# unknownue/puflow

Measured on AMD Instinct MI355X. Metric: patches/sec x4 2048->8192 (PU1K discrete, eval), higher is better.
Workload: dtype f32 (split-fp16 MFMA products, fp32 accumulate); 1 GPU; BASELINE configs[1]: PU1K discrete x4 inference, 32 x 2048-pt patches per GPU (fp32-parity mode); patches_per_gpu=32, total_batch=32, npoint=2048

## Files before the change

puflow_amd/csrc/edgeconv.hip:

```cpp
#include <hip/hip_runtime.h>
#include "pf_api_internal.h"
#include "pf_mfma.h"

namespace {

struct EcArgs {
    const float* pq;
    const float* xyz;
    const float* tab;
    const int* idx;
    const f4* wg;
    float* out;
    int T;
    int N;
    int chunk;
    int ntiles;
    const u4* pqf_w;
    const float* pqf_bias;
    const float* pqf_scales;
    float* pqf_out;
};

template <int ODIM>
__device__ __forceinline__ void pqf_stage(u4* hb, int ch, int pt, float v) {
// ... 328 lines not shown
            for (int o = 0; o < OCH; ++o)
#pragma unroll
                for (int p = 0; p < P; ++p)
                    m[p][ob0 + o] = fmaxf(fmaxf(acc[p][o].x, acc[p][o].y), fmaxf(acc[p][o].z, acc[p][o].w));
        });
#pragma unroll
        for (int p = 0; p < P; ++p) {
            const float o0 = pf_rsmax16(pf_rsmax32(m[p][0], m[p][1]), pf_rsmax32(m[p][2], m[p][3]));
            const float o1 = pf_rsmax16(pf_rsmax32(m[p][4], m[p][5]), pf_rsmax32(m[p][6], m[p][7]));
            const int ch = 16 * blkq + col;
            const float* pr = reinterpret_cast<const float*>(plds[wave * P + p]);
            const float p0 = pr[G * NCONV + ch], p1 = pr[G * NCONV + 64 + ch];
            const float h0 = fmaf(o0, EC4_OUT_INV, p0), h1 = fmaf(o1, EC4_OUT_INV, p1);
            if (pt0 + p < a.T) {
                float* o = a.out + (size_t)gout[p] * ODIM + ch;
                o[0] = h0;
                o[64] = h1;
            }
            if constexpr (PQF) {
                u4* hbt = hb + pqf.nst * ((ODIM / 32) * 2 * 64);
                pqf_stage<ODIM>(hbt, ch, wave * P + p, h0);
                pqf_stage<ODIM>(hbt, ch + 64, wave * P + p, h1);
            }
        }
        if constexpr (PQF) {
            pqf.push(pf_xcd_tile(v, a.chunk) * NW * P);
            if (pqf.nst == PQF_NT || vn >= vend) {
                __syncthreads();
                pqf_gemm<ODIM, 2 * S, NW>(a, hb, pqf.nst, pqf.tpt, __builtin_amdgcn_readfirstlane(wave), lane);
                __syncthreads();
                pqf.nst = 0;
            }
        }
        v = vn;
    }
}

template <int P, int NW, int DBG = 0, bool PQF = false>
int launch4(const EcArgs& a0, hipStream_t s) {
    EcArgs a = a0;
    a.ntiles = (a.T + NW * P - 1) / (NW * P);
    a.chunk = (a.ntiles + 7) / 8;
    int grid = 8 * a.chunk;
    if (grid > 256) grid = 256;
    hipLaunchKernelGGL((edgeconv4_kernel<P, NW, DBG, PQF>), dim3(grid), dim3(NW * 64), 0, s, a);
    return pf_last_launch_status();
}

template <int ODIM, bool C3, int P, int NW, bool PQF = false>
__global__ __launch_bounds__(NW * 64) void edgeconv1n_kernel(EcArgs a) {
    static_assert(!PQF || NW * P == 16, "the fused P|Q GEMM takes a workgroup tile of 16 points as one MFMA column tile");
    constexpr int NCONV = 4, S = 16 * NCONV + ODIM, SB = S / 16, OBO = ODIM / 16;
    constexpr int PQ_ROWS = ODIM == 32 ? 256 : 512;
    constexpr int FO = 4, FT = FO + OBO * 2, NWF = FT + (C3 ? SB : 0);
    constexpr int ROWB = 2 * S * 4;
    static_assert(OBO == 2 || OBO == 4, "reduce-scatter below is written for 2 or 4 output blocks");
    const int lane = threadIdx.x & 63, wave = threadIdx.x >> 6;
    const int col = lane & 15, q = lane >> 4;
    __shared__ u4 wlds[NWF * 128];
    __shared__ float plds[C3 ? 1 : NW * P][C3 ? 1 : S];
    __shared__ u4 hb[PQF ? PQF_NT * (ODIM / 32) * 2 * 64 : 1];
    PqfState pqf;
    pf_stage_lds(wlds, reinterpret_cast<const u4*>(a.wg), NWF * 128);
    __syncthreads();
    const PfW2Lds ws{wlds, lane};
    const __amdgpu_buffer_rsrc_t rs = __builtin_amdgcn_make_buffer_rsrc(const_cast<float*>(C3 ? a.xyz : a.pq), 0, 0x7fffffff, 0x00020000);

    for (int v = blockIdx.x; v < 8 * a.chunk; v += gridDim.x) {
        const int tile = pf_xcd_tile(v, a.chunk);
        if (tile >= a.ntiles) continue;
        const int pt0 = (tile * NW + wave) * P;
        int gi[P], vQ[P], vO[P][4];
        PfPairN e[P][1];
#pragma unroll
        for (int p = 0; p < P; ++p) {
            int g = pt0 + p;
            g = g < a.T ? g : a.T - 1;
            g = __builtin_amdgcn_readfirstlane(g);
            gi[p] = g;
            const int bN = (g / a.N) * a.N;
            const int jc = bN + a.idx[(size_t)g * 16 + col];
            if constexpr (C3) {
                float xi[3], xj[3];
#pragma unroll
                for (int c = 0; c < 3; ++c) {
                    xi[c] = a.xyz[(size_t)g * 3 + c];
                    xj[c] = a.xyz[(size_t)jc * 3 + c];
                }
                const f4 z4 = pf_splat(0.f);
                const f4 e0 = {xi[0], xi[1], xi[2], xj[0]}, e1 = {xj[1], xj[2], 0.f, 1.f};
                e[p][0] = pf_pairn(q == 0 ? e0 : z4, q == 0 ? e1 : z4);
            } else {
                const int4 j4 = *reinterpret_cast<const int4*>(a.idx + (size_t)g * 16 + 4 * q);
                vQ[p] = jc * ROWB + (S + 4 * q) * 4;
                vO[p][0] = (bN + j4.x) * ROWB + (S + 16 * NCONV + col) * 4;
                vO[p][1] = (bN + j4.y) * ROWB + (S + 16 * NCONV + col) * 4;
                vO[p][2] = (bN + j4.z) * ROWB + (S + 16 * NCONV + col) * 4;
                vO[p][3] = (bN + j4.w) * ROWB + (S + 16 * NCONV + col) * 4;
                if (lane * 2 < S) {
                    typedef float f2 __attribute__((ext_vector_type(2)));
                    const f2 pv = *reinterpret_cast<const f2*>(a.pq + (size_t)g * (2 * S) + lane * 2);
                    *reinterpret_cast<f2*>(&plds[wave * P + p][lane * 2]) = pv;
                }
            }
        }
        f4 pre[P][NCONV];
        f4 outi[P][OBO];
        if constexpr (C3) {
#pragma unroll
            for (int p = 0; p < P; ++p) {
#pragma unroll
                for (int b = 0; b < NCONV; ++b) pre[p][b] = pf_splat(0.f);
#pragma unroll
                for (int b = 0; b < OBO; ++b) outi[p][b] = pf_splat(0.f);
            }
            pf_mmn<false, NCONV, 1, 1>(ws, FT, e, pre);
            pf_mmn<true, OBO, 1, 1>(ws, FT + NCONV, e, outi);
        } else {
#pragma unroll
            for (int b = 0; b < NCONV; ++b)
#pragma unroll
                for (int p = 0; p < P; ++p)
                    pre[p][b] = __builtin_bit_cast(f4, __builtin_amdgcn_raw_buffer_load_b128(rs, vQ[p], b * 64, 0));
#pragma unroll
            for (int b = 0; b < OBO; ++b)
#pragma unroll
                for (int p = 0; p < P; ++p)
#pragma unroll
                    for (int r = 0; r < 4; ++r)
                        outi[p][b][r] = __builtin_bit_cast(float, __builtin_amdgcn_raw_buffer_load_b32(rs, vO[p][r], b * 64, 0));
#pragma unroll
            for (int b = 0; b < NCONV; ++b)
#pragma unroll
                for (int p = 0; p < P; ++p) pre[p][b] += *reinterpret_cast<const f4*>(&plds[wave * P + p][16 * b + 4 * q]);
        }

        PfPairN fp[P][2];
        f4 last[P];
#pragma unroll
        for (int p = 0; p < P; ++p) {
            last[p] = pf_lrelu(pre[p][0], 0.05f);
            fp[p][0] = pf_pairn(last[p], pf_splat(0.f));
        }
        pf_static_for<1, NCONV>([&](auto tc) {
            constexpr int t = decltype(tc)::value;
            constexpr int CPT = (t + 1) / 2, F0 = (t / 2) * ((t + 1) / 2);
            f4 acc[P][1];
#pragma unroll
            for (int p = 0; p < P; ++p) acc[p][0] = pre[p][t];
            pf_mmn<false, 1, CPT, CPT>(ws, F0, fp, acc);
#pragma unroll
            for (int p = 0; p < P; ++p) {
                const f4 f = pf_lrelu(acc[p][0], 0.05f);
                if constexpr (t % 2 == 1) fp[p][t / 2] = pf_pairn(last[p], f);
                else fp[p][t / 2] = pf_pairn(f, pf_splat(0.f));
                last[p] = f;
            }
        });
        pf_mmn<true, OBO, 2, 2>(ws, FO, fp, outi);
#pragma unroll
        for (int p = 0; p < P; ++p) {
            float m[OBO];
#pragma unroll
            for (int b = 0; b < OBO; ++b) m[b] = fmaxf(fmaxf(outi[p][b].x, outi[p][b].y), fmaxf(outi[p][b].z, outi[p][b].w));
            float o;
            int ch;
            if constexpr (OBO == 4) {
                o = pf_rsmax16(pf_rsmax32(m[0], m[1]), pf_rsmax32(m[2], m[3]));
                ch = 16 * (((q & 1) << 1) | (q >> 1)) + col;
            } else {
                const float n = pf_rsmax32(m[0], m[1]);
                o = pf_rsmax16(n, n);
                ch = 16 * (q >> 1) + col;
            }
            float pv = 0.f;
            if constexpr (!C3) pv = plds[wave * P + p][16 * NCONV + ch];
            const float hv = fmaf(o, EC4_OUT_INV, pv);
            if (pt0 + p < a.T && (OBO == 4 || (q & 1) == 0))
                a.out[(size_t)gi[p] * ODIM + ch] = hv;
            if constexpr (PQF) {
                if (OBO == 4 || (q & 1) == 0) pqf_stage<ODIM>(hb + pqf.nst * ((ODIM / 32) * 2 * 64), ch, wave * P + p, hv);
            }
        }
        if constexpr (PQF) {
            pqf.push(tile * NW * P);
            if (pqf.nst == PQF_NT) {
                __syncthreads();
                pqf_gemm<ODIM, PQ_ROWS, NW>(a, hb, pqf.nst, pqf.tpt, __builtin_amdgcn_readfirstlane(wave), lane);
                __syncthreads();
                pqf.nst = 0;
            }
        }
    }
    if constexpr (PQF) {
        if (pqf.nst > 0) {
            __syncthreads();
            pqf_gemm<ODIM, PQ_ROWS, NW>(a, hb, pqf.nst, pqf.tpt, __builtin_amdgcn_readfirstlane(wave), lane);
        }
    }
}

template <int ODIM, bool C3, int P, int NW, bool PQF = false>
int launch1n(const EcArgs& a0, hipStream_t s) {
// ... 152 lines not shown
```

puflow_amd/csrc/interp.hip:

```cpp
#include <hip/hip_runtime.h>
#include "pf_api_internal.h"
#include "pf_mfma.h"

#ifndef PF_INTERP_P
#define PF_INTERP_P 1
#endif
#ifndef PF_INTERP_NW
#define PF_INTERP_NW 12
#endif

namespace {

struct InterpArgs {
    const float* xyz;
    const float* z;
    const int* idx;
    const float* w;
    long long off[15];
    float* u;
    float* aw;
    int T, N, ntiles, R;
    int per;
    int contiguous;
};

template <int P, int NW, bool BIG = false>
__global__ __launch_bounds__(NW * 64) void interp_kernel(InterpArgs a) {
    constexpr int R = 4;
    const int lane = threadIdx.x & 63, wave = threadIdx.x >> 6;
    const int col = lane & 15, q = lane >> 4;
    const int ps = col >> 3, k = col & 7;
    constexpr int L_DT = 0, L_ET = 4, L_WT = 12, L_D3 = 20, L_EC = 28, L_D6 = 44, L_W3 = 60, L_END = 76;
    __shared__ u4 wl[L_END * 128];
    {
        auto stage = [&](int f0, int nf, long long off) {
            const u4* src = reinterpret_cast<const u4*>(a.w + off);
            pf_stage_lds(wl + f0 * 128, src, nf * 128);
        };
        if (a.contiguous) stage(L_DT, L_END, a.off[0]);
        else {
            stage(L_DT, 4, a.off[0]); stage(L_ET, 8, a.off[5]); stage(L_WT, 8, a.off[8]); stage(L_D3, 8, a.off[1]);
            stage(L_EC, 16, a.off[6]); stage(L_D6, 16, a.off[3]); stage(L_W3, 16, a.off[9]);
        }
        __syncthreads();
    }
    const PfW2Lds wsDT{wl + L_DT * 128, lane}, wsET{wl + L_ET * 128, lane}, wsWT{wl + L_WT * 128, lane},
        wsD3{wl + L_D3 * 128, lane}, wsEC{wl + L_EC * 128, lane}, wsD6{wl + L_D6 * 128, lane}, wsW3{wl + L_W3 * 128, lane};
    const PfW2BufD<4> wsW0(a.w + a.off[7], lane);
    const PfW2BufD<2> wsW6(a.w + a.off[BIG ? 13 : 11], lane);

    const float* sc = a.w + a.off[4];
    const float iDT = sc[0], iD3 = sc[1], iW1 = sc[2], iEC = sc[3], iW3 = sc[4], iW6 = sc[5];

    const int wt_end = min((int)(blockIdx.x + 1) * a.per, a.ntiles);
    for (int wt = blockIdx.x * a.per + wave; wt < wt_end; wt += NW) {
        const int pt0 = wt * P * 2;
        int gi[P], gj[P];
        bool ok[P];
        PfPairN e[P][1];
#pragma unroll
        for (int p = 0; p < P; ++p) {
            const int g = pt0 + p * 2 + ps;
            ok[p] = g < a.T;
            gi[p] = ok[p] ? g : a.T - 1;
            gj[p] = (gi[p] / a.N) * a.N + a.idx[(size_t)gi[p] * 16 + k];
            float xi[3], xj[3];
#pragma unroll
            for (int c = 0; c < 3; ++c) {
                xi[c] = a.xyz[(size_t)gi[p] * 3 + c];
                xj[c] = a.xyz[(size_t)gj[p] * 3 + c];
            }
            const float v0 = xi[0] - xj[0], v1 = xi[1] - xj[1], v2 = xi[2] - xj[2];
            const float nrm = sqrtf(__fadd_rn(__fadd_rn(__fmul_rn(v0, v0), __fmul_rn(v1, v1)), __fmul_rn(v2, v2)));
            const f4 z4 = pf_splat(0.f);
            const f4 e0 = {xi[0], xi[1], xi[2], xj[0]}, e1 = {xj[1], xj[2], nrm, 1.f};
            e[p][0] = pf_pairn(q == 0 ? e0 : z4, q == 0 ? e1 : z4);
        }

        f4 w1[P][8];
        {
            PfPairN fp[P][4];
            f4 last[P];
            {
                f4 acc[P][1];
#pragma unroll
                for (int p = 0; p < P; ++p) acc[p][0] = pf_splat(0.f);
                pf_mmn<false, 1, 1, 1>(wsET, 0, e, acc);
#pragma unroll
                for (int p = 0; p < P; ++p) {
                    last[p] = pf_lrelu(acc[p][0] * iEC, 0.05f);
                    fp[p][0] = pf_pairn(last[p], pf_splat(0.f));
                }
            }
            pf_static_for<1, 8>([&](auto tc) {
                constexpr int t = decltype(tc)::value;
                constexpr int CPT = (t + 1) / 2;
                constexpr int F0 = (t / 2) * ((t + 1) / 2);
                f4 acc[P][1];
#pragma unroll
                for (int p = 0; p < P; ++p) acc[p][0] = pf_splat(0.f);
                pf_mmn<false, 1, 1, 1>(wsET, t, e, acc);
                pf_mmn<false, 1, CPT, CPT>(wsEC, F0, fp, acc);
#pragma unroll
                for (int p = 0; p < P; ++p) {
                    const f4 f = pf_lrelu(acc[p][0] * iEC, 0.05f);
                    if constexpr (t % 2 == 1) fp[p][t / 2] = pf_pairn(last[p], f);
                    else fp[p][t / 2] = pf_pairn(f, pf_splat(0.f));
                    last[p] = f;
                }
            });
#pragma unroll
            for (int ob = 0; ob < 8; ++ob)
#pragma unroll
                for (int p = 0; p < P; ++p) w1[p][ob] = pf_splat(0.f);
            pf_mmn<false, 4, 1, 1>(wsWT, 0, e, w1, 0, 0);
            pf_mmn<false, 4, 1, 1>(wsWT, 4, e, w1, 0, 4);
            pf_mmn<false, 4, 4, 4>(wsW0, 0, fp, w1, 0, 0);
            pf_mmn<false, 4, 4, 4>(wsW0, 16, fp, w1, 0, 4);
        }

        {
            f4 d[P][4];
#pragma unroll
            for (int cb = 0; cb < 4; ++cb)
#pragma unroll
                for (int p = 0; p < P; ++p) d[p][cb] = pf_splat(0.f);
            pf_mmn<false, 4, 1, 1>(wsDT, 0, e, d);
            PfPairN dp[P][2];
#pragma unroll
            for (int p = 0; p < P; ++p) {
                dp[p][0] = pf_pairn(pf_lrelu(d[p][0] * iDT, 0.01f), pf_lrelu(d[p][1] * iDT, 0.01f));
                dp[p][1] = pf_pairn(pf_lrelu(d[p][2] * iDT, 0.01f), pf_lrelu(d[p][3] * iDT, 0.01f));
            }
#pragma unroll
            for (int cb = 0; cb < 4; ++cb)
#pragma unroll
                for (int p = 0; p < P; ++p) d[p][cb] = pf_bias(a.w + a.off[2], cb, q);
            pf_mmn<false, 4, 2, 2>(wsD3, 0, dp, d);
#pragma unroll
            for (int p = 0; p < P; ++p) {
                dp[p][0] = pf_pairn(pf_lrelu(d[p][0] * iD3, 0.01f), pf_lrelu(d[p][1] * iD3, 0.01f));
                dp[p][1] = pf_pairn(pf_lrelu(d[p][2] * iD3, 0.01f), pf_lrelu(d[p][3] * iD3, 0.01f));
            }
            pf_mmn<false, 4, 2, 2>(wsD6, 0, dp, w1, 0, 0);
            pf_mmn<false, 4, 2, 2>(wsD6, 8, dp, w1, 0, 4);
        }

        f4 w3[P][BIG ? 2 : 1];
        {
            PfPairN w1p[P][4];
#pragma unroll
            for (int c = 0; c < 4; ++c)
#pragma unroll
                for (int p = 0; p < P; ++p)
                    w1p[p][c] = pf_pairn(pf_lrelu(w1[p][2 * c] * iW1, 0.01f), pf_lrelu(w1[p][2 * c + 1] * iW1, 0.01f));
            f4 w2[P][4];
#pragma unroll
            for (int ob = 0; ob < 4; ++ob)
#pragma unroll
                for (int p = 0; p < P; ++p) w2[p][ob] = pf_bias(a.w + a.off[10], ob, q);
            pf_mmn<false, 4, 4, 4>(wsW3, 0, w1p, w2);
            PfPairN w2p[P][2];
#pragma unroll
            for (int p = 0; p < P; ++p) {
                w2p[p][0] = pf_pairn(pf_lrelu(w2[p][0] * iW3, 0.01f), pf_lrelu(w2[p][1] * iW3, 0.01f));
                w2p[p][1] = pf_pairn(pf_lrelu(w2[p][2] * iW3, 0.01f), pf_lrelu(w2[p][3] * iW3, 0.01f));
            }
#pragma unroll
            for (int p = 0; p < P; ++p)
#pragma unroll
                for (int ob = 0; ob < (BIG ? 2 : 1); ++ob) w3[p][ob] = pf_bias(a.w + a.off[BIG ? 14 : 12], ob, q);
            pf_mmn<false, (BIG ? 2 : 1), 2, 2>(wsW6, 0, w2p, w3);
#pragma unroll
            for (int p = 0; p < P; ++p)
#pragma unroll
                for (int ob = 0; ob < (BIG ? 2 : 1); ++ob) w3[p][ob] = w3[p][ob] * iW6;
        }

#pragma unroll
        for (int p = 0; p < P; ++p) {
// ... 11 lines not shown
                        m = fmaxf(m, __shfl_xor(m, 1)); m = fmaxf(m, __shfl_xor(m, 2)); m = fmaxf(m, __shfl_xor(m, 4));
                        const float ex = expf(x - m);
                        float sm = ex;
                        sm += __shfl_xor(sm, 1); sm += __shfl_xor(sm, 2); sm += __shfl_xor(sm, 4);
                        const float av = ex / sm;
#pragma unroll
                        for (int c = 0; c < 3; ++c) {
                            float s = av * zj[c];
                            s += __shfl_xor(s, 1); s += __shfl_xor(s, 2); s += __shfl_xor(s, 4);
                            if (ok[p] && k == 0 && row < a.R) a.u[((size_t)gi[p] * a.R + row) * 3 + c] = s;
                        }
                    }
            } else {
                float av[R];
#pragma unroll
                for (int r = 0; r < R; ++r) {
                    const float x = w3[p][0][r];
                    float m = x;
                    m = fmaxf(m, __shfl_xor(m, 1)); m = fmaxf(m, __shfl_xor(m, 2)); m = fmaxf(m, __shfl_xor(m, 4));
                    const float ex = expf(x - m);
                    float s = ex;
                    s += __shfl_xor(s, 1); s += __shfl_xor(s, 2); s += __shfl_xor(s, 4);
                    av[r] = ex / s;
                }
                if (a.aw) {
                    if (ok[p] && q == 0) {
                        f4 o = {av[0], av[1], av[2], av[3]};
                        *reinterpret_cast<f4*>(a.aw + ((size_t)gi[p] * 8 + k) * 4) = o;
                    }
                    continue;
                }
                const float zj = a.z[(size_t)gj[p] * 3 + (q < 3 ? q : 0)];
#pragma unroll
                for (int r = 0; r < R; ++r) {
                    float s = av[r] * zj;
                    s += __shfl_xor(s, 1); s += __shfl_xor(s, 2); s += __shfl_xor(s, 4);
                    if (ok[p] && k == 0 && q < 3 && r < a.R) a.u[((size_t)gi[p] * a.R + r) * 3 + q] = s;
                }
            }
        }
    }
}

}

static int interp_launch(const float* xyz, const float* z, const int* idx16, const float* w, const long long* off,
                         float* u_out, float* aw_out, int B, int N, int R, void* stream) {
    if (B <= 0 || N < 8 || (long long)B * N > (1ll << 28)) return PF_ERR_SHAPE;
    if (R < 1 || R > 32) return PF_ERR_UNSUPPORTED;
    constexpr int NWB = 8;
    InterpArgs a{};
    a.xyz = xyz; a.z = z; a.idx = idx16; a.w = w; a.u = u_out; a.aw = aw_out; a.T = B * N; a.N = N; a.R = R;
    for (int i = 0; i < 15; ++i) a.off[i] = off[i];
    a.contiguous = off[5] == off[0] + 4 * 512 && off[8] == off[5] + 8 * 512 && off[1] == off[8] + 8 * 512 &&
                   off[6] == off[1] + 8 * 512 && off[3] == off[6] + 16 * 512 && off[9] == off[3] + 16 * 512;
    auto go = [&](auto pc, auto nwc, auto bigc) {
        constexpr int P = decltype(pc)::value, NW = decltype(nwc)::value;
        constexpr bool BIG = decltype(bigc)::value;
        a.ntiles = (a.T + P * 2 - 1) / (P * 2);
        const int wgt = (a.ntiles + NW - 1) / NW;
        const int grid = wgt < 256 ? wgt : 256;
        a.per = (a.ntiles + grid - 1) / grid;
        hipLaunchKernelGGL((interp_kernel<P, NW, BIG>), dim3(grid), dim3(NW * 64), 0, (hipStream_t)stream, a);
    };
    if (R > 4) go(std::integral_constant<int, 1>{}, std::integral_constant<int, NWB>{}, std::true_type{});
    else go(std::integral_constant<int, PF_INTERP_P>{}, std::integral_constant<int, PF_INTERP_NW>{}, std::false_type{});
    return pf_last_launch_status();
}

extern "C" int pf_interp(const float* xyz, const float* z, const int* idx16, const float* w, const long long* off,
                         float* u_out, int B, int N, int R, void* stream) {
    if (!xyz || !z || !idx16 || !w || !off || !u_out) return PF_ERR_NULL;
    return interp_launch(xyz, z, idx16, w, off, u_out, nullptr, B, N, R, stream);
}

extern "C" int pf_interp_weights(const float* xyz, const int* idx16, const float* w, const long long* off, float* aw_out,
                                 int B, int N, void* stream) {
    if (!xyz || !idx16 || !w || !off || !aw_out) return PF_ERR_NULL;
    return interp_launch(xyz, nullptr, idx16, w, off, nullptr, aw_out, B, N, 4, stream);
}
```

puflow_amd/csrc/pf_mfma.h:

```cpp
#pragma once
#include <hip/hip_runtime.h>
#include <type_traits>

typedef float f4 __attribute__((ext_vector_type(4)));

#define PF_WAVE 64

__device__ __forceinline__ f4 pf_mfma(float a, float b, f4 c) {
    return __builtin_amdgcn_mfma_f32_16x16x4f32(a, b, c, 0, 0, 0);
}

__device__ __forceinline__ f4 pf_splat(float v) { f4 r = {v, v, v, v}; return r; }

__device__ __forceinline__ f4 pf_lrelu(f4 v, float slope) {
    const f4 s = v * slope;
    f4 r;
    r.x = fmaxf(v.x, s.x); r.y = fmaxf(v.y, s.y); r.z = fmaxf(v.z, s.z); r.w = fmaxf(v.w, s.w);
    return r;
}

__device__ __forceinline__ f4 pf_relu(f4 v) {
    f4 r;
    r.x = fmaxf(v.x, 0.f); r.y = fmaxf(v.y, 0.f); r.z = fmaxf(v.z, 0.f); r.w = fmaxf(v.w, 0.f);
    return r;
// ... 34 lines not shown
        if (i + DD < NFRAG) wb[i % DD] = ws.load(frag0 + ((i + DD) / CB) * WCB + ((i + DD) % CB));
#pragma unroll
        for (int r = 0; r < 4; ++r) {
#pragma unroll
            for (int p = 0; p < P; ++p)
                acc[p][acc0 + ob] = pf_mfma(wv[r], in[p][in0 + cb][r], acc[p][acc0 + ob]);
        }
        __builtin_amdgcn_sched_barrier(0);
    }
}

typedef unsigned int u4 __attribute__((ext_vector_type(4)));

typedef _Float16 h8 __attribute__((ext_vector_type(8)));
typedef _Float16 h2 __attribute__((ext_vector_type(2)));
typedef unsigned int u2 __attribute__((ext_vector_type(2)));
constexpr float PF_LO_SCALE = 2048.f, PF_LO_INV = 1.f / 2048.f;

__device__ __forceinline__ u2 pf_split2_pair(float a, float b) {
    unsigned hb = __builtin_bit_cast(unsigned, (h2){(_Float16)a, (_Float16)b});
    asm("" : "+v"(hb));
    const h2 h = __builtin_bit_cast(h2, hb);
    const h2 l = {(_Float16)((a - (float)h.x) * PF_LO_SCALE), (_Float16)((b - (float)h.y) * PF_LO_SCALE)};
    return (u2){hb, __builtin_bit_cast(unsigned, l)};
}

struct PfPair2 { h8 h, l; };
__device__ __forceinline__ PfPair2 pf_pair2(f4 b0, f4 b1) {
    const u2 s0 = pf_split2_pair(b0.x, b0.y), s1 = pf_split2_pair(b0.z, b0.w);
    const u2 s2 = pf_split2_pair(b1.x, b1.y), s3 = pf_split2_pair(b1.z, b1.w);
    PfPair2 p;
    p.h = __builtin_bit_cast(h8, (u4){s0.x, s1.x, s2.x, s3.x});
    p.l = __builtin_bit_cast(h8, (u4){s0.y, s1.y, s2.y, s3.y});
    return p;
}

__device__ __forceinline__ f4 pf_mfma_f16(h8 a, h8 b, f4 c) {
    return __builtin_amdgcn_mfma_f32_16x16x32_f16(a, b, c, 0, 0, 0);
}

#ifndef PF_MM2_DEPTH
#define PF_MM2_DEPTH 8
#endif
#ifndef PF_W2LDS_DEPTH
#define PF_W2LDS_DEPTH 2
#endif
struct PfW2Lds {
    static constexpr int DEPTH = PF_W2LDS_DEPTH;
    const u4* base;
    int lane;
    __device__ __forceinline__ h8 load(int frag, int split) const {
        return __builtin_bit_cast(h8, base[(frag * 2 + split) * PF_WAVE + lane]);
    }
};

template <int DEPTH_>
struct PfW2BufD {
    static constexpr int DEPTH = DEPTH_;
    __amdgpu_buffer_rsrc_t rsrc;
    int voff;
    __device__ __forceinline__ PfW2BufD(const void* p, int lane)
        : rsrc(__builtin_amdgcn_make_buffer_rsrc(const_cast<void*>(p), 0, 0x7fffffff, 0x00020000)), voff(lane * 16) {}
    __device__ __forceinline__ h8 load(int frag, int split) const {
        return __builtin_bit_cast(h8, __builtin_amdgcn_raw_buffer_load_b128(rsrc, voff, (frag * 2 + split) * (PF_WAVE * 16), 0));
    }
};

struct PfW2Buf {
    static constexpr int DEPTH = PF_MM2_DEPTH;
    __amdgpu_buffer_rsrc_t rsrc;
    int voff;
    __device__ __forceinline__ PfW2Buf(const void* p, int lane)
        : rsrc(__builtin_amdgcn_make_buffer_rsrc(const_cast<void*>(p), 0, 0x7fffffff, 0x00020000)), voff(lane * 16) {}
    __device__ __forceinline__ h8 load(int frag, int split) const {
        return __builtin_bit_cast(h8, __builtin_amdgcn_raw_buffer_load_b128(rsrc, voff, (frag * 2 + split) * (PF_WAVE * 16), 0));
    }
};

template <int OB, int CP, int WCP, int D = 2, class WS2, int P, int NIN, int NACC>
__device__ __forceinline__ void pf_mm2(const WS2& ws, int frag0, const PfPair2 (&in)[P][NIN], int in0,
                                       f4 (&acc)[P][NACC], f4 (&accx)[P][NACC], int acc0) {
    constexpr int NFRAG = OB * CP;
    constexpr int DD = D < NFRAG ? D : NFRAG;
    h8 wb[DD][2];
#pragma unroll
    for (int i = 0; i < DD; ++i)
#pragma unroll
        for (int s = 0; s < 2; ++s) wb[i][s] = ws.load(frag0 + (i / CP) * WCP + (i % CP), s);
#pragma unroll
    for (int i = 0; i < NFRAG; ++i) {
        const int ob = i / CP, cp = i % CP;
        const h8 wh = wb[i % DD][0], wl = wb[i % DD][1];
        if (i + DD < NFRAG) {
            const int f = frag0 + ((i + DD) / CP) * WCP + ((i + DD) % CP);
#pragma unroll
            for (int s = 0; s < 2; ++s) wb[i % DD][s] = ws.load(f, s);
        }
#pragma unroll
        for (int p = 0; p < P; ++p) {
            f4 x = accx[p][acc0 + ob];
            x = pf_mfma_f16(wh, in[p][in0 + cp].l, x);
            x = pf_mfma_f16(wl, in[p][in0 + cp].h, x);
            accx[p][acc0 + ob] = x;
            acc[p][acc0 + ob] = pf_mfma_f16(wh, in[p][in0 + cp].h, acc[p][acc0 + ob]);
        }
        __builtin_amdgcn_sched_barrier(0);
// ... 68 lines not shown
#endif
#ifndef PF_MMN_PRIO
#define PF_MMN_PRIO 0
#endif
template <bool SWAP, int OB, int CP, int WCP, bool FENCE = true, class WS, int P, int NIN, int NACC>
__device__ __forceinline__ void pf_mmn(const WS& ws, int frag0, const PfPairN (&feat)[P][NIN], f4 (&acc)[P][NACC], int in0 = 0, int acc0 = 0) {
    constexpr int D = WS::DEPTH;
    constexpr int NFRAG = OB * CP;
    constexpr int DD = D < NFRAG ? D : NFRAG;
    auto OBI = [](int i) { return PF_MMN_CPMAJOR ? i % OB : i / CP; };
    auto CPI = [](int i) { return PF_MMN_CPMAJOR ? i / OB : i % CP; };
    h8 wb[DD][2];
#pragma unroll
    for (int i = 0; i < DD; ++i)
#pragma unroll
        for (int s = 0; s < 2; ++s) wb[i][s] = ws.load(frag0 + OBI(i) * WCP + CPI(i), s);
#if PF_MMN_PRIO
    __builtin_amdgcn_s_setprio(PF_MMN_PRIO);
#endif
#pragma unroll
    for (int i = 0; i < NFRAG; ++i) {
        const int ob = OBI(i), cp = CPI(i);
        const h8 wh = wb[i % DD][0], wl = wb[i % DD][1];
        if (i + DD < NFRAG) {
            const int f = frag0 + OBI(i + DD) * WCP + CPI(i + DD);
#pragma unroll
            for (int s = 0; s < 2; ++s) wb[i % DD][s] = ws.load(f, s);
        }
#pragma unroll
        for (int p = 0; p < P; ++p) {
            f4 x = acc[p][acc0 + ob];
            if constexpr (SWAP) {
                if constexpr (PF_MMN_TERMS == 3) {
                    x = pf_mfma_f16(feat[p][in0 + cp].l, wh, x);
                    x = pf_mfma_f16(feat[p][in0 + cp].h, wl, x);
                }
                x = pf_mfma_f16(feat[p][in0 + cp].h, wh, x);
            } else {
                if constexpr (PF_MMN_TERMS == 3) {
                    x = pf_mfma_f16(wh, feat[p][in0 + cp].l, x);
                    x = pf_mfma_f16(wl, feat[p][in0 + cp].h, x);
                }
                x = pf_mfma_f16(wh, feat[p][in0 + cp].h, x);
            }
            acc[p][acc0 + ob] = x;
        }
        if constexpr (FENCE) __builtin_amdgcn_sched_barrier(0);
    }
#if PF_MMN_PRIO
    __builtin_amdgcn_s_setprio(0);
#endif
}


template <int D = 8, class T4>
__device__ __forceinline__ void pf_stage_lds(T4* __restrict__ dst, const T4* __restrict__ src, int n) {
    const int nt = blockDim.x;
    for (int base = threadIdx.x; base < n; base += nt * D) {
        T4 v[D];
#pragma unroll
        for (int k = 0; k < D; ++k) {
            const int i = base + k * nt;
            v[k] = src[i < n ? i : n - 1];
        }
#pragma unroll
        for (int k = 0; k < D; ++k) {
            const int i = base + k * nt;
            if (i < n) dst[i] = v[k];
        }
    }
}

template <int I, int N, class F>
__device__ __forceinline__ void pf_static_for(F&& f) {
    if constexpr (I < N) {
        f(std::integral_constant<int, I>{});
        pf_static_for<I + 1, N>(f);
    }
}

__device__ __forceinline__ f4 pf_bias(const float* __restrict__ b, int ob, int q) {
    return *reinterpret_cast<const f4*>(b + ob * 16 + 4 * q);
}

__device__ __forceinline__ float pf_rowmax16(float v) {
    v = fmaxf(v, __builtin_bit_cast(float, __builtin_amdgcn_update_dpp(0, __builtin_bit_cast(int, v), 0x128, 0xf, 0xf, false)));
    v = fmaxf(v, __builtin_bit_cast(float, __builtin_amdgcn_update_dpp(0, __builtin_bit_cast(int, v), 0x124, 0xf, 0xf, false)));
    v = fmaxf(v, __builtin_bit_cast(float, __builtin_amdgcn_update_dpp(0, __builtin_bit_cast(int, v), 0x122, 0xf, 0xf, false)));
    v = fmaxf(v, __builtin_bit_cast(float, __builtin_amdgcn_update_dpp(0, __builtin_bit_cast(int, v), 0x121, 0xf, 0xf, false)));
    return v;
}

__device__ __forceinline__ int pf_xcd_tile(int v, int chunk) { return (v & 7) * chunk + (v >> 3); }
```

puflow_amd/packing.py:

```python
from __future__ import annotations

from typing import Dict, List

import numpy as np

NUM_BLOCKS = 6
FEAT_CHANNELS = [3, 32, 64, 128, 128, 128, 128]
GROWTH = [8, 16, 32, 32, 32, 32]
COND_CHANNELS = [32, 64, 128, 128, 128, 128]
HDIM = 64
BN_EPS = 1e-5


def _np(sd, k):
    return sd[k].detach().cpu().numpy().astype(np.float64)


def _fold_bn(sd, conv: str, bn: str):
    W = _np(sd, conv + ".weight")
    W = W.reshape(W.shape[0], -1)
    b = _np(sd, conv + ".bias")
    s = _np(sd, bn + ".weight") / np.sqrt(_np(sd, bn + ".running_var") + BN_EPS)
    return W * s[:, None], s * (b - _np(sd, bn + ".running_mean")) + _np(sd, bn + ".bias")

# ... 108 lines not shown

def frag_pack(W: np.ndarray) -> np.ndarray:
    out, inn = W.shape
    OB, CB = (out + 15) // 16, (inn + 15) // 16
    Wp = np.zeros((OB * 16, CB * 16), dtype=np.float32)
    Wp[:out, :inn] = W
    f = Wp.reshape(OB, 16, CB, 4, 4)
    return np.ascontiguousarray(f.transpose(0, 2, 3, 1, 4)).reshape(OB, CB, 64, 4)


F16_LO_SCALE = 2048.0


def frag_pack_f16x2(W: np.ndarray) -> np.ndarray:
    out, inn = W.shape
    OB, CP = (out + 15) // 16, (inn + 31) // 32
    Wp = np.zeros((OB * 16, CP * 32), dtype=np.float32)
    Wp[:out, :inn] = W
    if np.abs(Wp).max(initial=0.0) >= 65504.0:
        raise ValueError("weight magnitude exceeds the fp16 range of the f16x2 path; use ec_mode='f32'")
    hi = Wp.astype(np.float16)
    lo = ((Wp - hi.astype(np.float32)).astype(np.float32) * np.float32(F16_LO_SCALE)).astype(np.float16)
    lanes = np.arange(64)
    row, q = lanes & 15, lanes >> 4
    j = np.arange(8)
    ch = np.where(j[None, :] < 4, 4 * q[:, None] + j[None, :], 16 + 4 * q[:, None] + (j[None, :] - 4))
    res = np.zeros((OB, CP, 2, 64, 8), dtype=np.uint16)
    for si, part in enumerate((hi, lo)):
        bits = part.view(np.uint16).reshape(OB, 16, CP, 32)
        res[:, :, si] = bits.reshape(OB, 16, CP, 2, 4, 4).transpose(0, 2, 4, 1, 3, 5).reshape(OB, CP, 64, 8)
    return res.reshape(-1).view(np.float32)


def frag_pack_f16n(W: np.ndarray) -> np.ndarray:
    out, inn = W.shape
    OB, CP = (out + 15) // 16, (inn + 31) // 32
    Wp = np.zeros((OB * 16, CP * 32), dtype=np.float32)
    Wp[:out, :inn] = W
    if np.abs(Wp).max(initial=0.0) >= 65504.0:
        raise ValueError("scaled weight magnitude exceeds the fp16 range of the f16n path; use ec_mode='f32'")
    hi = Wp.astype(np.float16)
    lo = (Wp - hi.astype(np.float32)).astype(np.float32).astype(np.float16)
    lanes = np.arange(64)
    row, q = lanes & 15, lanes >> 4
    j = np.arange(8)
    ch = np.where(j[None, :] < 4, 4 * q[:, None] + j[None, :], 16 + 4 * q[:, None] + (j[None, :] - 4))
    res = np.zeros((OB, CP, 2, 64, 8), dtype=np.uint16)
    for si, part in enumerate((hi, lo)):
        bits = part.view(np.uint16).reshape(OB, 16, CP, 32)
        res[:, :, si] = bits.reshape(OB, 16, CP, 2, 4, 4).transpose(0, 2, 4, 1, 3, 5).reshape(OB, CP, 64, 8)
    return res.reshape(-1).view(np.float32)


def f16n_scale(W: np.ndarray) -> float:
    m = float(np.abs(W).max(initial=0.0))
    if m == 0.0 or not np.isfinite(m):
        return 1.0
    return float(2.0 ** int(np.clip(13 - np.floor(np.log2(m)), -24, 40)))


def frag_pack_f16n_scaled(W: np.ndarray):
    sc = f16n_scale(W)
    return frag_pack_f16n((W.astype(np.float64) * sc).astype(np.float32)), np.float32(1.0 / sc)


EC4_STEP = 4.0


def ec4_scales(nconv: int = 4, g: int = 32, odim: int = 128):
    a = EC4_STEP ** np.arange(nconv + 1)
    S = g * nconv + odim
    rp = np.ones(S); rq = np.ones(S)
    for t in range(nconv):
        rp[g * t:g * (t + 1)] = a[t]; rq[g * t:g * (t + 1)] = a[t]
    rq[g * nconv:] = a[nconv]
    return rp.astype(np.float32), rq.astype(np.float32), a.astype(np.float32)


def ec4_weights(u: Dict[str, np.ndarray], nconv: int = 4, g: int = 32) -> np.ndarray:
    _, _, a = ec4_scales(nconv, g, u[f"G{nconv}"].shape[0])
    parts = []
    for t in range(1, nconv + 1):
        Gt = u[f"G{t}"].astype(np.float64).copy()
        for c in range(t):
            Gt[:, g * c:g * (c + 1)] *= a[t] / a[c]
        parts.append(frag_pack_f16n(Gt.astype(np.float32)))
    return np.concatenate(parts)


def frag_unpack_f16x2(F: np.ndarray, out: int, inn: int) -> np.ndarray:
    OB, CP = (out + 15) // 16, (inn + 31) // 32
    img = np.ascontiguousarray(F, dtype=np.float32).view(np.uint16).reshape(OB, CP, 2, 64, 8).view(np.float16).astype(np.float64)
    val = img[:, :, 0] + img[:, :, 1] / F16_LO_SCALE
    lanes = np.arange(64)
    row, q = lanes & 15, lanes >> 4
    j = np.arange(8)
    ch = np.where(j[None, :] < 4, 4 * q[:, None] + j[None, :], 16 + 4 * q[:, None] + (j[None, :] - 4))
    W = np.zeros((OB, 16, CP, 32))
    W[:, row[:, None], :, ch] = val.transpose(2, 3, 0, 1)
    return W.reshape(OB * 16, CP * 32)[:out, :inn]


def frag_unpack_f16n(F: np.ndarray, out: int, inn: int) -> np.ndarray:
    OB, CP = (out + 15) // 16, (inn + 31) // 32
    img = np.ascontiguousarray(F, dtype=np.float32).view(np.uint16).reshape(OB, CP, 2, 64, 8).view(np.float16).astype(np.float64)
    val = img[:, :, 0] + img[:, :, 1]
    lanes = np.arange(64)
    row, q = lanes & 15, lanes >> 4
    j = np.arange(8)
    ch = np.where(j[None, :] < 4, 4 * q[:, None] + j[None, :], 16 + 4 * q[:, None] + (j[None, :] - 4))
    W = np.zeros((OB, 16, CP, 32))
    W[:, row[:, None], :, ch] = val.transpose(2, 3, 0, 1)
    return W.reshape(OB * 16, CP * 32)[:out, :inn]


def frag_unpack(F: np.ndarray, out: int, inn: int) -> np.ndarray:
    OB, CB = F.shape[0], F.shape[1]
    f = F.reshape(OB, CB, 4, 16, 4).transpose(0, 3, 1, 2, 4)
    return f.reshape(OB * 16, CB * 16)[:out, :inn]


POST_SLOTS = ["M1", "b1", "M2", "H1", "S2", "bS2", "T2", "bT2", "ST4", "bST4", "PQ", "bPQ", "scales"]
POST_SCALES = ["M1", "M2", "H1", "S2", "T2", "ST4", "PQ"]
INTERP_SLOTS = ["dtab", "d_W3", "d_b3", "d_W6", "scales", "ectab", "ec_w", "w_W0", "w_b0", "w_W3", "w_b3", "w_W6", "w_b6",
                "w_W6full", "w_b6full"]
INTERP_SCALES = ["dtab", "d_W3", "w1", "ec", "w_W3", "w_W6"]
FLOW_REC = 5360


class _Blob:
    def __init__(self):
        self.parts: List[np.ndarray] = []
        self.n = 0

    def add(self, a: np.ndarray) -> int:
        a = np.ascontiguousarray(a, dtype=np.float32).reshape(-1)
        off = self.n
        pad = (-a.size) % 64
        self.parts.append(a)
# ... 31 lines not shown
    return W


def _etab_frag(xi: np.ndarray, xj: np.ndarray, nrm, const: np.ndarray) -> np.ndarray:
    rows = xi.shape[0]
    W = np.zeros((rows, 32), np.float32)
    W[:, 0:3] = xi
    W[:, 3] = xj[:, 0]
    W[:, 16:18] = xj[:, 1:3]
    if nrm is not None:
        W[:, 18] = nrm
    W[:, 19] = const
    return frag_pack_f16x2(W)


def _ec_frags(u: Dict[str, np.ndarray], nconv: int) -> np.ndarray:
    return np.concatenate([frag_pack(u[f"G{t}"]).reshape(-1) for t in range(1, nconv + 1)])


def pack_flow_record(f: Dict[str, object]) -> np.ndarray:
    rec = np.zeros(FLOW_REC, np.float32)
    img2, inv2 = frag_pack_f16n_scaled(f["c1_W2"])
    rec[0:4096] = img2
    W4 = f["c1_W4"]
    W4r = np.zeros((16, 64), np.float32)
    b4r = np.zeros(16, np.float32)
    for q in range(4):
        W4r[4 * q:4 * q + W4.shape[0]] = W4
        b4r[4 * q:4 * q + W4.shape[0]] = f["c1_b4"]
    img4, inv4 = frag_pack_f16n_scaled(W4r)
    rec[4096:5120] = img4
    rec[5120:5184] = f["c1_b2"] / inv2
    rec[5184:5200] = b4r / inv4
    W0h = np.zeros((64, 2), np.float32)
    W0h[:, :f["tdim"]] = f["c1_W0h"]
    rec[5200:5328] = W0h.reshape(-1)
    rec[5328:5337] = f["A"].reshape(-1); rec[5337:5340] = f["a0"]
    rec[5340:5349] = f["Ai"].reshape(-1); rec[5349:5352] = f["ai0"]
    rec[5352], rec[5353] = inv2, inv4
    return rec


def pack_plan(plan: Dict[str, object], ec_mode: str = "f16n") -> Dict[str, object]:
    if ec_mode not in ("f16n", "f32"):
        raise ValueError(f"unknown EdgeConv arithmetic mode {ec_mode!r}")
    B = _Blob()
    out: Dict[str, object] = {}
    units = plan["units"]
    out["ec_tab0"] = B.add(_edge_table(units[0]))
    out["ec_w"] = [B.add(_ec_frags(units[i], 4)) for i in range(NUM_BLOCKS)]
    out["ec4_w"] = [None, None] + [B.add(ec4_weights(units[i])) for i in range(2, NUM_BLOCKS)]
    ec1n = []
    for i in range(2):
        parts = [ec4_weights(units[i], 4, 16)]
        if i == 0:
            rp, rq, _ = ec4_scales(4, 16, 32)
            parts.append(frag_pack_f16n(_etab_dense(units[0]["PA"] * rq[:, None], units[0]["QB"] * rq[:, None], None, units[0]["pb"] * rq)))
        ec1n.append(B.add(np.concatenate(parts)))
    out["ec1n_w"] = ec1n + [None] * (NUM_BLOCKS - 2)
    out["ec_mode"] = ec_mode
    post = []
    for i in range(NUM_BLOCKS):
        m, f = plan["merges"][i], plan["flows"][i]
        H1 = (np.concatenate([f["s_W0"], f["t_W0"], f["c1_W0c"]], axis=0).astype(np.float64)
              @ m["W2"].astype(np.float64)).astype(np.float32)
        ST4 = np.zeros((6, 128), np.float32)
        ST4[0:3, 0:64] = f["s_W4"]; ST4[3:6, 64:128] = f["t_W4"]
        bST4 = _pad_vec(np.concatenate([f["s_b4"], f["t_b4"]]), 16)
        inv = {}
        def img(name, W):
            im, inv[name] = frag_pack_f16n_scaled(W)
            return B.add(im)
        offs = {"M1": img("M1", m["W1"]), "H1": img("H1", H1), "S2": img("S2", f["s_W2"]), "T2": img("T2", f["t_W2"]),
                "ST4": img("ST4", ST4)}
        assert offs["ST4"] + 4 * 512 == B.n and (B.n - offs["M1"]) % 512 == 0
        offs["M2"] = img("M2", m["W2"])
        offs["b1"] = B.add(_pad_vec(m["b1"], ((m["b1"].size + 15) // 16) * 16) / inv["M1"])
        offs["bS2"] = B.add(f["s_b2"] / inv["S2"]); offs["bT2"] = B.add(f["t_b2"] / inv["T2"])
        offs["bST4"] = B.add(bST4 / inv["ST4"])
        if i + 1 < NUM_BLOCKS:
            nu = units[i + 1]
            Wpq = np.concatenate([nu["PA"], nu["QB"]], axis=0)
            bpq = np.concatenate([nu["pb"], np.zeros_like(nu["pb"])])
            if ec_mode == "f16n":
                rp, rq, _ = ec4_scales() if i + 1 >= 2 else ec4_scales(4, 16, 64)
                rs = np.concatenate([rp, rq])
                Wpq, bpq = Wpq * rs[:, None], bpq * rs
            offs["PQ"] = img("PQ", Wpq)
            offs["bPQ"] = B.add(bpq)
        else:
            offs["PQ"], offs["bPQ"], inv["PQ"] = 0, 0, np.float32(1.0)
        offs["scales"] = B.add(_pad_vec(np.array([inv[k] for k in POST_SCALES], np.float32), 16))
        post.append([offs[k] for k in POST_SLOTS])
    out["post"] = post
    out["flow"] = B.add(np.concatenate([pack_flow_record(f) for f in plan["flows"]]))
    out["ld_const"] = float(sum(f["ld_const"] for f in plan["flows"]))
    ip = plan["interp"]
    W6r = np.zeros((16, 64), np.float32)
    b6r = np.zeros(16, np.float32)
    for q in range(4):
        W6r[4 * q:4 * q + 4] = ip["w_W6"][:4]
        b6r[4 * q:4 * q + 4] = ip["w_b6"][:4]
    ec = ip["ec"]
    ft = ip["f_tab"]
    def grp(*mats):
        sc = min(f16n_scale(m) for m in mats)
        return sc, [frag_pack_f16n((m.astype(np.float64) * sc).astype(np.float32)) for m in mats]
    dtab_d = _etab_dense(ip["d_PA"], ip["d_QB"], ip["d_wn"], ip["d_b0"])
    ectab_d = _etab_dense(ec["PA"][:128], ec["QB"][:128], None, ec["pb"][:128])
    w1tab_d = _etab_dense(ft[:, 0:3], ft[:, 3:6], None, ft[:, 6] + ip["f_b0"])
    s_dt, (i_dt,) = grp(dtab_d)
    s_d3, (i_d3,) = grp(ip["d_W3"])
    s_w1, (i_w1t, i_d6, i_w0) = grp(w1tab_d, ip["f_dW"], ip["f_eW"])
    ecG = [ec[f"G{t}"] for t in range(1, 8)]
    s_ec, ec_imgs = grp(ectab_d, *ecG)
    s_w3, (i_w3,) = grp(ip["w_W3"])
    s_w6, (i_w6r, i_w6f) = grp(W6r, ip["w_W6"])
    io = {}
    for k, im in (("dtab", i_dt), ("ectab", ec_imgs[0]), ("w_b0", i_w1t), ("d_W3", i_d3), ("ec_w", np.concatenate(ec_imgs[1:])),
                  ("d_W6", i_d6), ("w_W3", i_w3)):
        io[k] = B.add(im)
    assert B.n - io["dtab"] == 76 * 512
    io.update({
        "d_b3": B.add(ip["d_b3"] * s_d3),
        "scales": B.add(_pad_vec(np.array([1 / s_dt, 1 / s_d3, 1 / s_w1, 1 / s_ec, 1 / s_w3, 1 / s_w6], np.float32), 16)),
        "w_W0": B.add(i_w0),
        "w_b3": B.add(ip["w_b3"] * s_w3),
        "w_W6": B.add(i_w6r), "w_b6": B.add(b6r * s_w6),
        "w_W6full": B.add(i_w6f), "w_b6full": B.add(ip["w_b6"] * s_w6),
    })
    out["interp"] = [io[k] for k in INTERP_SLOTS]
    out["blob"] = B.data()
    return out


CNF_REC = 10160
CNF_CTX = 288


def _np32(t) -> np.ndarray:
    return t.detach().cpu().numpy().astype(np.float32) if hasattr(t, "detach") else np.asarray(t, np.float32)


LOG2E = 1.4426950408889634


def pack_cnf_context(Hc: np.ndarray):
    return frag_pack_f16n_scaled(np.ascontiguousarray(Hc, dtype=np.float32))


def cnf_split_ok(rec, T_end: float) -> bool:
    tv = np.asarray(rec[9872:9872 + CNF_CTX], np.float64)
    g = np.concatenate([tv[0:64], tv[128:192], tv[256:272]])
    return bool(np.abs(g).max() * abs(T_end) <= 100.0)


def pack_cnf_block(sd, i: int):
    p = f"flow_blocks.{i}.cnf.odefunc.diffeq.layers"
    L = [{k: _np32(sd[f"{p}.{j}.{k}"]) for k in ("_layer.weight", "_layer.bias", "_hyper_bias.weight",
                                               "_hyper_gate.weight", "_hyper_gate.bias")} for j in range(3)]
    cdim = L[0]["_hyper_gate.weight"].shape[1] - 1
    Hc = np.zeros((CNF_CTX, cdim), np.float32)
    hb = np.zeros(CNF_CTX, np.float32)
    tv = np.zeros(CNF_CTX, np.float32)

    def put(row0, Wg, bg, rep):
        rows = Wg.shape[0]
        for qq in range(4 if rep else 1):
            r0 = row0 + 4 * qq if rep else row0
            Hc[r0:r0 + rows] = Wg[:, 1:]
            tv[r0:r0 + rows] = Wg[:, 0]
            if bg is not None:
                hb[r0:r0 + rows] = bg

    put(0, L[0]["_hyper_gate.weight"], L[0]["_hyper_gate.bias"], False)
# ... 30 lines not shown
```

Before: 27020 patches/s.

## Pack sparse-K split-fp16 MFMA operands to cut MFMA count in EdgeConv and interp

Input edge features that occupy only k-slots 0..7 are now packed so the hi/lo split terms share one MFMA (kpack8). Odd-stage conv blocks whose last K pair is half-empty get the same treatment (kpack16), which folds two split products into a single MFMA. Weight images are repacked on the host to match, which also shrinks the LDS weight footprint for interp and edgeconv1n. The aim is fewer MFMA issues and weight loads per point, at the cost of more complex packing invariants that must stay consistent between the host packer and the kernel.

```diff
diff --git a/puflow_amd/csrc/edgeconv.hip b/puflow_amd/csrc/edgeconv.hip
--- a/puflow_amd/csrc/edgeconv.hip
+++ b/puflow_amd/csrc/edgeconv.hip
@@ -404,7 +404,7 @@
     static_assert(!PQF || NW * P == 16, "the fused P|Q GEMM takes a workgroup tile of 16 points as one MFMA column tile");
     constexpr int NCONV = 4, S = 16 * NCONV + ODIM, SB = S / 16, OBO = ODIM / 16;
     constexpr int PQ_ROWS = ODIM == 32 ? 256 : 512;
-    constexpr int FO = 4, FT = FO + OBO * 2, NWF = FT + (C3 ? SB : 0);
+    constexpr int FO = 4, FT = FO + OBO * 2, NWF = FT + (C3 ? SB / 2 : 0);
     constexpr int ROWB = 2 * S * 4;
     static_assert(OBO == 2 || OBO == 4, "reduce-scatter below is written for 2 or 4 output blocks");
     const int lane = threadIdx.x & 63, wave = threadIdx.x >> 6;
@@ -423,7 +423,7 @@
         if (tile >= a.ntiles) continue;
         const int pt0 = (tile * NW + wave) * P;
         int gi[P], vQ[P], vO[P][4];
-        PfPairN e[P][1];
+        h8 e[P];
 #pragma unroll
         for (int p = 0; p < P; ++p) {
             int g = pt0 + p;
@@ -439,9 +439,8 @@
                     xi[c] = a.xyz[(size_t)g * 3 + c];
                     xj[c] = a.xyz[(size_t)jc * 3 + c];
                 }
-                const f4 z4 = pf_splat(0.f);
                 const f4 e0 = {xi[0], xi[1], xi[2], xj[0]}, e1 = {xj[1], xj[2], 0.f, 1.f};
-                e[p][0] = pf_pairn(q == 0 ? e0 : z4, q == 0 ? e1 : z4);
+                e[p] = pf_kpack8(pf_pairn(e0, e1), q);
             } else {
                 const int4 j4 = *reinterpret_cast<const int4*>(a.idx + (size_t)g * 16 + 4 * q);
                 vQ[p] = jc * ROWB + (S + 4 * q) * 4;
@@ -466,8 +465,8 @@
 #pragma unroll
                 for (int b = 0; b < OBO; ++b) outi[p][b] = pf_splat(0.f);
             }
-            pf_mmn<false, NCONV, 1, 1>(ws, FT, e, pre);
-            pf_mmn<true, OBO, 1, 1>(ws, FT + NCONV, e, outi);
+            pf_mmk8<false, NCONV>(ws, 2 * FT, e, pre);
+            pf_mmk8<true, OBO>(ws, 2 * FT + NCONV, e, outi);
         } else {
 #pragma unroll
             for (int b = 0; b < NCONV; ++b)
@@ -500,7 +499,11 @@
             f4 acc[P][1];
 #pragma unroll
             for (int p = 0; p < P; ++p) acc[p][0] = pre[p][t];
-            pf_mmn<false, 1, CPT, CPT>(ws, F0, fp, acc);
+            if constexpr (t % 2 == 0) pf_mmn<false, 1, CPT, CPT>(ws, F0, fp, acc);
+            else {
+                if constexpr (CPT > 1) pf_mmn<false, 1, CPT - 1, CPT>(ws, F0, fp, acc);
+                pf_mmk16<false, 1, CPT>(ws, F0 + CPT - 1, fp, CPT - 1, acc);
+            }
 #pragma unroll
             for (int p = 0; p < P; ++p) {
                 const f4 f = pf_lrelu(acc[p][0], 0.05f);
diff --git a/puflow_amd/csrc/interp.hip b/puflow_amd/csrc/interp.hip
--- a/puflow_amd/csrc/interp.hip
+++ b/puflow_amd/csrc/interp.hip
@@ -30,7 +30,7 @@
     const int lane = threadIdx.x & 63, wave = threadIdx.x >> 6;
     const int col = lane & 15, q = lane >> 4;
     const int ps = col >> 3, k = col & 7;
-    constexpr int L_DT = 0, L_ET = 4, L_WT = 12, L_D3 = 20, L_EC = 28, L_D6 = 44, L_W3 = 60, L_END = 76;
+    constexpr int L_DT = 0, L_ET = 2, L_WT = 6, L_D3 = 10, L_EC = 18, L_D6 = 34, L_W3 = 50, L_END = 66;
     __shared__ u4 wl[L_END * 128];
     {
         auto stage = [&](int f0, int nf, long long off) {
@@ -39,7 +39,7 @@
         };
         if (a.contiguous) stage(L_DT, L_END, a.off[0]);
         else {
-            stage(L_DT, 4, a.off[0]); stage(L_ET, 8, a.off[5]); stage(L_WT, 8, a.off[8]); stage(L_D3, 8, a.off[1]);
+            stage(L_DT, 2, a.off[0]); stage(L_ET, 4, a.off[5]); stage(L_WT, 4, a.off[8]); stage(L_D3, 8, a.off[1]);
             stage(L_EC, 16, a.off[6]); stage(L_D6, 16, a.off[3]); stage(L_W3, 16, a.off[9]);
         }
         __syncthreads();
@@ -57,7 +57,7 @@
         const int pt0 = wt * P * 2;
         int gi[P], gj[P];
         bool ok[P];
-        PfPairN e[P][1];
+        h8 e[P];
 #pragma unroll
         for (int p = 0; p < P; ++p) {
             const int g = pt0 + p * 2 + ps;
@@ -72,9 +72,8 @@
             }
             const float v0 = xi[0] - xj[0], v1 = xi[1] - xj[1], v2 = xi[2] - xj[2];
             const float nrm = sqrtf(__fadd_rn(__fadd_rn(__fmul_rn(v0, v0), __fmul_rn(v1, v1)), __fmul_rn(v2, v2)));
-            const f4 z4 = pf_splat(0.f);
             const f4 e0 = {xi[0], xi[1], xi[2], xj[0]}, e1 = {xj[1], xj[2], nrm, 1.f};
-            e[p][0] = pf_pairn(q == 0 ? e0 : z4, q == 0 ? e1 : z4);
+            e[p] = pf_kpack8(pf_pairn(e0, e1), q);
         }
 
         f4 w1[P][8];
@@ -85,7 +84,7 @@
                 f4 acc[P][1];
 #pragma unroll
                 for (int p = 0; p < P; ++p) acc[p][0] = pf_splat(0.f);
-                pf_mmn<false, 1, 1, 1>(wsET, 0, e, acc);
+                pf_mmk8<false, 1>(wsET, 0, e, acc);
 #pragma unroll
                 for (int p = 0; p < P; ++p) {
                     last[p] = pf_lrelu(acc[p][0] * iEC, 0.05f);
@@ -99,8 +98,12 @@
                 f4 acc[P][1];
 #pragma unroll
                 for (int p = 0; p < P; ++p) acc[p][0] = pf_splat(0.f);
-                pf_mmn<false, 1, 1, 1>(wsET, t, e, acc);
-                pf_mmn<false, 1, CPT, CPT>(wsEC, F0, fp, acc);
+                pf_mmk8<false, 1>(wsET, t, e, acc);
+                if constexpr (t % 2 == 0) pf_mmn<false, 1, CPT, CPT>(wsEC, F0, fp, acc);
+                else {
+                    if constexpr (CPT > 1) pf_mmn<false, 1, CPT - 1, CPT>(wsEC, F0, fp, acc);
+                    pf_mmk16<false, 1, CPT>(wsEC, F0 + CPT - 1, fp, CPT - 1, acc);
+                }
 #pragma unroll
                 for (int p = 0; p < P; ++p) {
                     const f4 f = pf_lrelu(acc[p][0] * iEC, 0.05f);
@@ -113,8 +116,8 @@
             for (int ob = 0; ob < 8; ++ob)
 #pragma unroll
                 for (int p = 0; p < P; ++p) w1[p][ob] = pf_splat(0.f);
-            pf_mmn<false, 4, 1, 1>(wsWT, 0, e, w1, 0, 0);
-            pf_mmn<false, 4, 1, 1>(wsWT, 4, e, w1, 0, 4);
+            pf_mmk8<false, 4>(wsWT, 0, e, w1, 0);
+            pf_mmk8<false, 4>(wsWT, 4, e, w1, 4);
             pf_mmn<false, 4, 4, 4>(wsW0, 0, fp, w1, 0, 0);
             pf_mmn<false, 4, 4, 4>(wsW0, 16, fp, w1, 0, 4);
         }
@@ -125,7 +128,7 @@
             for (int cb = 0; cb < 4; ++cb)
 #pragma unroll
                 for (int p = 0; p < P; ++p) d[p][cb] = pf_splat(0.f);
-            pf_mmn<false, 4, 1, 1>(wsDT, 0, e, d);
+            pf_mmk8<false, 4>(wsDT, 0, e, d);
             PfPairN dp[P][2];
 #pragma unroll
             for (int p = 0; p < P; ++p) {
@@ -243,7 +246,7 @@
     InterpArgs a{};
     a.xyz = xyz; a.z = z; a.idx = idx16; a.w = w; a.u = u_out; a.aw = aw_out; a.T = B * N; a.N = N; a.R = R;
     for (int i = 0; i < 15; ++i) a.off[i] = off[i];
-    a.contiguous = off[5] == off[0] + 4 * 512 && off[8] == off[5] + 8 * 512 && off[1] == off[8] + 8 * 512 &&
+    a.contiguous = off[5] == off[0] + 2 * 512 && off[8] == off[5] + 4 * 512 && off[1] == off[8] + 4 * 512 &&
                    off[6] == off[1] + 8 * 512 && off[3] == off[6] + 16 * 512 && off[9] == off[3] + 16 * 512;
     auto go = [&](auto pc, auto nwc, auto bigc) {
         constexpr int P = decltype(pc)::value, NW = decltype(nwc)::value;
diff --git a/puflow_amd/csrc/pf_mfma.h b/puflow_amd/csrc/pf_mfma.h
--- a/puflow_amd/csrc/pf_mfma.h
+++ b/puflow_amd/csrc/pf_mfma.h
@@ -110,6 +110,7 @@
     __device__ __forceinline__ h8 load(int frag, int split) const {
         return __builtin_bit_cast(h8, base[(frag * 2 + split) * PF_WAVE + lane]);
     }
+    __device__ __forceinline__ h8 load1(int frag) const { return __builtin_bit_cast(h8, base[frag * PF_WAVE + lane]); }
 };
 
 template <int DEPTH_>
@@ -284,6 +285,60 @@
 #endif
 }
 
+__device__ __forceinline__ h8 pf_kpack8(const PfPairN& x, int q) {
+    const u4 z = {0u, 0u, 0u, 0u};
+    const u4 h = __builtin_bit_cast(u4, x.h), l = __builtin_bit_cast(u4, x.l);
+    u4 r;
+    if constexpr (PF_MMN_TERMS == 3) r = q == 1 ? l : (q == 3 ? z : h);
+    else r = q == 0 ? h : z;
+    return __builtin_bit_cast(h8, r);
+}
+
+template <bool SWAP, int OB, class WS, int P, int NACC>
+__device__ __forceinline__ void pf_mmk8(const WS& ws, int frag0, const h8 (&x)[P], f4 (&acc)[P][NACC], int acc0 = 0) {
+    constexpr int DD = WS::DEPTH < OB ? WS::DEPTH : OB;
+    h8 wb[DD];
+#pragma unroll
+    for (int i = 0; i < DD; ++i) wb[i] = ws.load1(frag0 + i);
+#pragma unroll
+    for (int ob = 0; ob < OB; ++ob) {
+        const h8 w = wb[ob % DD];
+        if (ob + DD < OB) wb[ob % DD] = ws.load1(frag0 + ob + DD);
+#pragma unroll
+        for (int p = 0; p < P; ++p)
+            acc[p][acc0 + ob] = SWAP ? pf_mfma_f16(x[p], w, acc[p][acc0 + ob]) : pf_mfma_f16(w, x[p], acc[p][acc0 + ob]);
+        __builtin_amdgcn_sched_barrier(0);
+    }
+}
+
+__device__ __forceinline__ h8 pf_kpack16(const PfPairN& x) {
+    const u4 h = __builtin_bit_cast(u4, x.h), l = __builtin_bit_cast(u4, x.l);
+    return __builtin_bit_cast(h8, (u4){h.x, h.y, l.x, l.y});
+}
+
+template <bool SWAP, int OB, int WCP, class WS, int P, int NIN, int NACC>
+__device__ __forceinline__ void pf_mmk16(const WS& ws, int frag0, const PfPairN (&feat)[P][NIN], int cp, f4 (&acc)[P][NACC],
+                                         int acc0 = 0) {
+#pragma unroll
+    for (int ob = 0; ob < OB; ++ob) {
+        const h8 wd = ws.load(frag0 + ob * WCP, 0);
+#pragma unroll
+        for (int p = 0; p < P; ++p) {
+            f4 x = acc[p][acc0 + ob];
+            if constexpr (PF_MMN_TERMS == 3) {
+                const h8 wl = ws.load(frag0 + ob * WCP, 1);
+                const h8 xp = pf_kpack16(feat[p][cp]);
+                x = SWAP ? pf_mfma_f16(feat[p][cp].h, wl, x) : pf_mfma_f16(wl, feat[p][cp].h, x);
+                x = SWAP ? pf_mfma_f16(xp, wd, x) : pf_mfma_f16(wd, xp, x);
+            } else {
+                x = SWAP ? pf_mfma_f16(feat[p][cp].h, wd, x) : pf_mfma_f16(wd, feat[p][cp].h, x);
+            }
+            acc[p][acc0 + ob] = x;
+        }
+        __builtin_amdgcn_sched_barrier(0);
+    }
+}
+
 
 template <int D = 8, class T4>
 __device__ __forceinline__ void pf_stage_lds(T4* __restrict__ dst, const T4* __restrict__ src, int n) {
diff --git a/puflow_amd/packing.py b/puflow_amd/packing.py
--- a/puflow_amd/packing.py
+++ b/puflow_amd/packing.py
@@ -184,6 +184,24 @@
     return res.reshape(-1).view(np.float32)
 
 
+def kpack8_f16n(img: np.ndarray) -> np.ndarray:
+    a = np.ascontiguousarray(img, dtype=np.float32).view(np.uint16).reshape(-1, 2, 4, 16, 8)
+    if np.any(a[:, :, 1:]):
+        raise ValueError("k8 packing needs an operand block that uses only k-slots 0..7")
+    res = np.zeros((a.shape[0], 4, 16, 8), np.uint16)
+    res[:, 0] = res[:, 1] = a[:, 0, 0]
+    res[:, 2] = a[:, 1, 0]
+    return res.reshape(-1).view(np.float32)
+
+
+def kpack16_f16n(img: np.ndarray, OB: int, CP: int, cp: int) -> np.ndarray:
+    a = np.ascontiguousarray(img, dtype=np.float32).view(np.uint16).reshape(OB, CP, 2, 64, 8).copy()
+    if np.any(a[:, cp, :, :, 4:]):
+        raise ValueError("k16 packing needs a block pair whose second block is empty")
+    a[:, cp, 0, :, 4:] = a[:, cp, 0, :, :4]
+    return a.reshape(-1).view(np.float32)
+
+
 def f16n_scale(W: np.ndarray) -> float:
     m = float(np.abs(W).max(initial=0.0))
     if m == 0.0 or not np.isfinite(m):
@@ -209,14 +227,18 @@
     return rp.astype(np.float32), rq.astype(np.float32), a.astype(np.float32)
 
 
-def ec4_weights(u: Dict[str, np.ndarray], nconv: int = 4, g: int = 32) -> np.ndarray:
+def ec4_weights(u: Dict[str, np.ndarray], nconv: int = 4, g: int = 32, k16: bool = False) -> np.ndarray:
     _, _, a = ec4_scales(nconv, g, u[f"G{nconv}"].shape[0])
     parts = []
     for t in range(1, nconv + 1):
         Gt = u[f"G{t}"].astype(np.float64).copy()
         for c in range(t):
             Gt[:, g * c:g * (c + 1)] *= a[t] / a[c]
-        parts.append(frag_pack_f16n(Gt.astype(np.float32)))
+        im = frag_pack_f16n(Gt.astype(np.float32))
+        if k16 and (g * t) % 32 == 16:
+            OB, CP = (Gt.shape[0] + 15) // 16, (g * t + 31) // 32
+            im = kpack16_f16n(im, OB, CP, CP - 1)
+        parts.append(im)
     return np.concatenate(parts)
 
 
@@ -354,10 +376,11 @@
     out["ec4_w"] = [None, None] + [B.add(ec4_weights(units[i])) for i in range(2, NUM_BLOCKS)]
     ec1n = []
     for i in range(2):
-        parts = [ec4_weights(units[i], 4, 16)]
+        parts = [ec4_weights(units[i], 4, 16, k16=True)]
         if i == 0:
             rp, rq, _ = ec4_scales(4, 16, 32)
-            parts.append(frag_pack_f16n(_etab_dense(units[0]["PA"] * rq[:, None], units[0]["QB"] * rq[:, None], None, units[0]["pb"] * rq)))
+            parts.append(kpack8_f16n(frag_pack_f16n(_etab_dense(units[0]["PA"] * rq[:, None], units[0]["QB"] * rq[:, None], None,
+                                                                units[0]["pb"] * rq))))
         ec1n.append(B.add(np.concatenate(parts)))
     out["ec1n_w"] = ec1n + [None] * (NUM_BLOCKS - 2)
     out["ec_mode"] = ec_mode
@@ -416,13 +439,16 @@
     s_w1, (i_w1t, i_d6, i_w0) = grp(w1tab_d, ip["f_dW"], ip["f_eW"])
     ecG = [ec[f"G{t}"] for t in range(1, 8)]
     s_ec, ec_imgs = grp(ectab_d, *ecG)
+    i_dt, i_w1t, ec_imgs[0] = kpack8_f16n(i_dt), kpack8_f16n(i_w1t), kpack8_f16n(ec_imgs[0])
+    for t in range(1, 8, 2):
+        ec_imgs[t] = kpack16_f16n(ec_imgs[t], 1, (t + 1) // 2, (t - 1) // 2)
     s_w3, (i_w3,) = grp(ip["w_W3"])
     s_w6, (i_w6r, i_w6f) = grp(W6r, ip["w_W6"])
     io = {}
     for k, im in (("dtab", i_dt), ("ectab", ec_imgs[0]), ("w_b0", i_w1t), ("d_W3", i_d3), ("ec_w", np.concatenate(ec_imgs[1:])),
                   ("d_W6", i_d6), ("w_W3", i_w3)):
         io[k] = B.add(im)
-    assert B.n - io["dtab"] == 76 * 512
+    assert B.n - io["dtab"] == 66 * 512
     io.update({
         "d_b3": B.add(ip["d_b3"] * s_d3),
         "scales": B.add(_pad_vec(np.array([1 / s_dt, 1 / s_d3, 1 / s_w1, 1 / s_ec, 1 / s_w3, 1 / s_w6], np.float32), 16)),
```

New measurement: 27340 patches/s, median of 6. 1.01x the previous value.
